# xarray-contrib/xeofs

Measured on AMD Instinct MI355X. Metric: EOF randomized-SVD GB/s (algorithmic: 16 passes x n x p x 4 B per fit / fit time), higher is better.
Workload: dtype f32 data, split-fp16 MFMA (f16x3+f16x3), f32 accumulate

## Files before the change

### xeofs_amd/csrc/eofx_abi.hip

```cpp
#include <chrono>
#include "eofx_hfft.hpp"
#include "eofx_kernels.hpp"
#include "eofx_fit.hpp"
#include "eofx_gram.hpp"
#include "eofx_axb_dma.hpp"
#include "eofx_hosteig.hpp"
#include "eofx_hostla.hpp"
#include "eofx_lag.hpp"
#include "eofx_gw.hpp"
#include "eofx_spca.hpp"
#include "eofx_lagcov.hpp"
#include "eofx_lowpass.hpp"
#include "eofx_orderpos.hpp"
#include "eofx_colquad.hpp"
#include "eofx_pairmin.hpp"
#include "eofx_spectral.hpp"
#include "eofx_pcmul.hpp"
#include "eofx_viewcov.hpp"
#include "eofx_lrfill.hpp"
#include "eofx_plans.hpp"
#include "eofx_sketch.hpp"
#include "eofx_hilbert_host.hpp"
#include "eofx_gwplan.hpp"
#ifndef EOFX_AXB_DMA_DEFAULT
#define EOFX_AXB_DMA_DEFAULT 1
#endif

#include <algorithm>
#include <array>
#include <atomic>
#include <cmath>
#include <complex>
#include <cstdarg>
#include <cstdio>
#include <cstring>
#include <functional>
#include <string>
#include <thread>
#include <mutex>
#include <shared_mutex>
#include <condition_variable>
#include <deque>
#include <memory>
#include <vector>

#include <dlfcn.h>
#include <pthread.h>
#include <sched.h>
#include <hipfft/hipfft.h>

#include "eofx.h"

using namespace eofx;

struct ncclUniqueIdCompat {
  char internal[128];
};

struct EofxComm {
  int world = 1, rank = 0;
  void* lib = nullptr;
  void* comm = nullptr;
  int (*p_allreduce)(const void*, void*, size_t, int, int, void*, hipStream_t) = nullptr;
  int (*p_destroy)(void*) = nullptr;
  const char* (*p_errstr)(int) = nullptr;
  eofx_allreduce_fn fn = nullptr;
  void* user = nullptr;
  int64_t calls = 0, bytes = 0;
  std::vector<std::pair<hipEvent_t, hipEvent_t>> events;
};

struct eofx_ctx {
  int device = 0;
  hipStream_t stream = nullptr;
  char* arena = nullptr;
  size_t arena_size = 0;
  size_t arena_off = 0;
  std::string err;
  int prec_power = EOFX_PREC_F16X3;
  int prec_final = EOFX_PREC_F16X3;
  std::vector<std::pair<void*, size_t>> pool;
  size_t pool_bytes = 0;
  size_t pool_cap = (size_t)160 << 30;
  struct HilbertSetup {
    int64_t n = 0, P = 0;
    int padding = 0;
    double decay = 0.0;
    void* chat = nullptr;
    float* hperm = nullptr;
    float* u = nullptr;
  };
  std::vector<HilbertSetup> hsetups;
  struct HilbertOp {
    int64_t n = 0;
    int padding = 0;
    double decay = 0.0;
    eofx_mat* m = nullptr;
  };
  std::vector<HilbertOp> hops;
  std::vector<std::pair<std::pair<int64_t, int64_t>, std::pair<void*, void*>>> fft_plans;
  int keep_raw = 0;
  bool allow_masked = false;
  bool want_rawT = false;
  float* pending_rawT = nullptr;
  size_t pending_rawT_bytes = 0;
  bool profile = false;
  struct ProfEvent {
    hipEvent_t first, second;
    int kind;
    ProfEvent(hipEvent_t a, hipEvent_t b, int k = 0) : first(a), second(b), kind(k) {}
  };
  std::vector<ProfEvent> prof_events;
  int64_t prof_kind_launches[3] = {0, 0, 0};
  double prof_kind_ms[3] = {0.0, 0.0, 0.0};
  double prof_flops = 0.0;
  double prof_bytes = 0.0;
  unsigned* amax_slots = nullptr;
  int amax_next = 0, amax_depth = 0;
  std::vector<std::pair<const float*, const unsigned*>> amax_known;
  double* pinned = nullptr;
  struct GramPlanDev {
    int nti = 0, ntj = 0, nst = 0;
    bool sym = false;
    GramPlan pl;
    GramItem* items = nullptr;
    int2* tiles = nullptr;
  };
  std::vector<GramPlanDev*> gram_plans;
  _Float16* axb_planes = nullptr;
  size_t axb_planes_bytes = 0;
  int axb_dma = -1;
  double fit_info[4] = {0.0, 0.0, 0.0, 0.0};
  int last_iters = 0;
  EofxComm* comm = nullptr;
};
constexpr int EOFX_AMAX_SLOTS = 1024;
constexpr int EOFX_HILBERT_OP_MAX_N = 16384;
constexpr size_t EOFX_PINNED_DOUBLES = 2 * 256 * 256 + 64;

struct eofx_mat {
  int64_t n = 0, p = 0, n_pad = 0, p_pad = 0;
  float* X = nullptr;
  float* Xt = nullptr;
  const float* raw = nullptr;
  float* raw_owned = nullptr;
  size_t raw_owned_bytes = 0;
  int64_t raw_ld = 0;
  float* aff = nullptr;
  unsigned* absmax_dev = nullptr;
  float absmax = 0.f;
  bool masked = false;
  int64_t p_valid = 0;
  int* act = nullptr;
  int64_t n_act = -1;
  float* rawT = nullptr;
};

static int set_err(eofx_ctx* ctx, int code, const char* fmt, ...) {
  char buf[512];
  va_list ap;
  va_start(ap, fmt);
  vsnprintf(buf, sizeof(buf), fmt, ap);
  va_end(ap);
  if (ctx) ctx->err = buf;
  return code;
}

#define HIPCHK(expr)                                                                          \
  do {                                                                                        \
    hipError_t _e = (expr);                                                                   \
    if (_e != hipSuccess)                                                                     \
      return set_err(ctx, _e == hipErrorOutOfMemory ? EOFX_ERR_NOMEM : EOFX_ERR_HIP,           \
                     "%s failed: %s (%s:%d)", #expr, hipGetErrorString(_e), __FILE__, __LINE__); \
// ... 92 lines not shown
    if (excl) {
      (void)hipStreamSynchronize(ctx->stream);
      g_fence[dev].mu.unlock();
    } else {
      g_fence[dev].mu.unlock_shared();
    }
  }
};
#define ENTER(c)          \
  FenceGuard _fence((c), false); \
  CHK(set_device(c))
#define ENTER_EXCLUSIVE(c)      \
  FenceGuard _fence((c), true); \
  CHK(set_device(c))

extern "C" int eofx_abi_version(void) { return EOFX_ABI_VERSION; }

extern "C" int eofx_ctx_create(int device, void* stream, eofx_ctx** out) {
  if (!out) return EOFX_ERR_ARG;
  eofx_ctx* ctx = new eofx_ctx();
  ctx->device = device;
  ctx->stream = (hipStream_t)stream;
  hipError_t e = hipSetDevice(device);
  if (e != hipSuccess) {
    delete ctx;
    *out = nullptr;
    return EOFX_ERR_HIP;
  }
  if (device >= 0 && device < EOFX_MAX_DEVICES) {
    std::lock_guard<std::mutex> g(g_fence[device].reg_mu);
    g_fence[device].ctxs.push_back(ctx);
  }
  *out = ctx;
  return EOFX_OK;
}
extern "C" int eofx_ctx_destroy(eofx_ctx* ctx) {
  if (!ctx) return EOFX_OK;
  {
    FenceGuard fence(ctx, false);
    if (ctx->device >= 0 && ctx->device < EOFX_MAX_DEVICES) {
      std::lock_guard<std::mutex> g(g_fence[ctx->device].reg_mu);
      auto& v = g_fence[ctx->device].ctxs;
      v.erase(std::remove(v.begin(), v.end(), ctx), v.end());
    }
  }
  (void)hipSetDevice(ctx->device);
  if (ctx->arena) {
    (void)hipStreamSynchronize(ctx->stream);
    (void)hipFree(ctx->arena);
  }
  pool_trim(ctx);
  if (ctx->amax_slots) (void)hipFree(ctx->amax_slots);
  if (ctx->pinned) (void)hipHostFree(ctx->pinned);
  for (auto& e : ctx->fft_plans) {
    hipfftDestroy((hipfftHandle)e.second.first);
    hipfftDestroy((hipfftHandle)e.second.second);
  }
  (void)eofx_ctx_comm_clear(ctx);
  if (ctx->axb_planes) (void)hipFree(ctx->axb_planes);
  for (auto* g : ctx->gram_plans) {
    if (g->items) (void)hipFree(g->items);
    if (g->tiles) (void)hipFree(g->tiles);
    delete g;
  }
  for (auto& h : ctx->hops) (void)eofx_mat_destroy(ctx, h.m);
  ctx->hops.clear();
  for (auto& h : ctx->hsetups) {
    if (h.chat) (void)hipFree(h.chat);
    if (h.hperm) (void)hipFree(h.hperm);
    if (h.u) (void)hipFree(h.u);
  }
  delete ctx;
  return EOFX_OK;
}
extern "C" int eofx_ctx_set_stream(eofx_ctx* ctx, void* stream) {
  if (!ctx) return EOFX_ERR_ARG;
  ENTER(ctx);
  if ((hipStream_t)stream == ctx->stream) return EOFX_OK;
  HIPCHK(hipStreamSynchronize(ctx->stream));
  ctx->stream = (hipStream_t)stream;
  for (auto& e : ctx->fft_plans) {
    if (hipfftSetStream((hipfftHandle)e.second.first, ctx->stream) != HIPFFT_SUCCESS ||
        hipfftSetStream((hipfftHandle)e.second.second, ctx->stream) != HIPFFT_SUCCESS)
      return set_err(ctx, EOFX_ERR_HIP, "hipfftSetStream failed while moving the context to another stream");
  }
  return EOFX_OK;
}
extern "C" int eofx_ctx_synchronize(eofx_ctx* ctx) {
  if (!ctx) return EOFX_ERR_ARG;
  ENTER(ctx);
  HIPCHK(hipStreamSynchronize(ctx->stream));
  return EOFX_OK;
}
extern "C" const char* eofx_last_error(const eofx_ctx* ctx) { return ctx ? ctx->err.c_str() : ""; }

extern "C" int eofx_ctx_profile(eofx_ctx* ctx, int enable) {
  if (!ctx) return EOFX_ERR_ARG;
  ctx->profile = enable != 0;
  return EOFX_OK;
}
extern "C" int eofx_ctx_profile_read(eofx_ctx* ctx, int64_t* launches, double* total_ms, double* flops,
                                     double* bytes) {
  if (!ctx) return EOFX_ERR_ARG;
  ENTER(ctx);
  HIPCHK(hipStreamSynchronize(ctx->stream));
  double ms = 0.0;
// ... 17 lines not shown
  ctx->prof_events.clear();
  ctx->prof_flops = 0.0;
  ctx->prof_bytes = 0.0;
  return EOFX_OK;
}

extern "C" int eofx_ctx_profile_by_kernel(const eofx_ctx* ctx, int64_t* launches3, double* ms3) {
  if (!ctx) return EOFX_ERR_ARG;
  for (int k = 0; k < 3; ++k) {
    if (launches3) launches3[k] = ctx->prof_kind_launches[k];
    if (ms3) ms3[k] = ctx->prof_kind_ms[k];
  }
  return EOFX_OK;
}

static int copy_out(eofx_ctx* ctx, void* dst, const void* src_dev, size_t bytes) {
  if (!dst || bytes == 0) return EOFX_OK;
  HIPCHK(hipMemcpyAsync(dst, src_dev, bytes, hipMemcpyDefault, ctx->stream));
  return EOFX_OK;
}
static int copy_in(eofx_ctx* ctx, void* dst_dev, const void* src, size_t bytes) {
  if (bytes == 0) return EOFX_OK;
  HIPCHK(hipMemcpyAsync(dst_dev, src, bytes, hipMemcpyDefault, ctx->stream));
  return EOFX_OK;
}

struct AmaxScope {
  eofx_ctx* ctx;
  explicit AmaxScope(eofx_ctx* c) : ctx(c) {
    if (ctx->amax_depth++ == 0) {
      ctx->amax_known.clear();
      ctx->amax_next = 0;
      if (!ctx->amax_slots && hipMalloc((void**)&ctx->amax_slots, sizeof(unsigned) * EOFX_AMAX_SLOTS) != hipSuccess) {
        (void)hipGetLastError();
        ctx->amax_slots = nullptr;
      }
      if (ctx->amax_slots &&
          hipMemsetAsync(ctx->amax_slots, 0, sizeof(unsigned) * EOFX_AMAX_SLOTS, ctx->stream) != hipSuccess) {
        (void)hipGetLastError();
        ctx->amax_next = EOFX_AMAX_SLOTS;
      }
    }
  }
  ~AmaxScope() {
    if (--ctx->amax_depth == 0) ctx->amax_known.clear();
  }
};
static void amax_forget(eofx_ctx* ctx, const float* panel) {
  for (size_t i = 0; i < ctx->amax_known.size(); ++i)
    if (ctx->amax_known[i].first == panel) {
      ctx->amax_known.erase(ctx->amax_known.begin() + i);
      return;
    }
}
static unsigned* amax_new(eofx_ctx* ctx, const float* panel) {
  if (ctx->amax_depth == 0) return nullptr;
  amax_forget(ctx, panel);
  if (!ctx->amax_slots || ctx->amax_next >= EOFX_AMAX_SLOTS) return nullptr;
  unsigned* slot = ctx->amax_slots + ctx->amax_next++;
  ctx->amax_known.emplace_back(panel, slot);
  return slot;
}
static const float* amax_get(const eofx_ctx* ctx, const float* panel) {
  if (ctx->amax_depth == 0) return nullptr;
  for (auto& e : ctx->amax_known)
    if (e.first == panel) return reinterpret_cast<const float*>(e.second);
  return nullptr;
}
static int pinned_scratch(eofx_ctx* ctx, double** out) {
  if (!ctx->pinned) HIPCHK(hipHostMalloc((void**)&ctx->pinned, sizeof(double) * EOFX_PINNED_DOUBLES, hipHostMallocDefault));
  *out = ctx->pinned;
  return EOFX_OK;
}

extern "C" int eofx_host_zheigh_top_f64(const double* Hr, const double* Hi, int m, int nev, double* w, double* Xr, double* Xi) {
  if (!Hr || !Hi || !w || !Xr || !Xi || m <= 0 || nev <= 0 || nev > m) return EOFX_ERR_ARG;
  return hosteig::zheigh_top(Hr, Hi, m, nev, w, Xr, Xi) == 0 ? EOFX_OK : EOFX_ERR_LINALG;
}
extern "C" int eofx_host_eigh_f64(const double* Ain, int n, double* w, double* Vec) {
  if (!Ain || !w || !Vec || n <= 0) return EOFX_ERR_ARG;
  return hosteig::eigh(Ain, n, w, Vec) == 0 ? EOFX_OK : EOFX_ERR_LINALG;
}


struct AffView {
  const float* aff = nullptr;
  int64_t ld = 0;
  int rows = 0;
  int64_t cols = 0;
  bool masked = false;
};
template <int NB>
static void launch_atb_variant(int prec, dim3 grid, hipStream_t st, const float* A, int64_t lda,
                               const float* B, int ldb, float* out, int L, int64_t M, int64_t K,
                               int64_t kps, int col_base, float a_scale, const float* b_absmax,
                               const AffView* aff = nullptr, const float* A2 = nullptr, const float* B2 = nullptr,
                               int s_half = 0, int sym = 0, unsigned* amax_out = nullptr, int l_valid = 128) {
  if (prec == EOFX_PREC_F16X3 && A2)
    hipLaunchKernelGGL(atb_f16_kernel<NB>, grid, dim3(256), 0, st, A, lda, B, ldb, out, L, M, K, kps, col_base,
                       a_scale, b_absmax, (const float*)nullptr, (int64_t)0, 0, (int64_t)0, A2, B2, s_half, 0, amax_out, l_valid);
  else if (prec == EOFX_PREC_F16X3 && aff && aff->masked)
    hipLaunchKernelGGL((atb_f16_kernel<NB, true, true>), grid, dim3(256), 0, st, A, lda, B, ldb, out, L, M, K, kps, col_base,
                       a_scale, b_absmax, aff->aff, aff->ld, aff->rows, aff->cols, (const float*)nullptr, (const float*)nullptr, 0, sym, amax_out,
                       l_valid);
  else if (prec == EOFX_PREC_F16X3 && aff)
    hipLaunchKernelGGL((atb_f16_kernel<NB, true>), grid, dim3(256), 0, st, A, lda, B, ldb, out, L, M, K, kps, col_base,
// ... 3283 lines not shown
};

static bool cplx_lean(const eofx_mat* A, const eofx_mat* B, int LP, int prec_power, int prec_final) {
  const bool all_written = A->X && A->Xt && B->X && B->Xt;
  return !all_written && !B->masked && LP == 64 && prec_power == EOFX_PREC_F16X3 && prec_final == EOFX_PREC_F16X3;
}
static int cplx_lean_setup(eofx_ctx* ctx, CplxOps& ops) {
  const int64_t n = ops.A->n, il = round_up(n, AXB_KG);
  float* ident = arena_alloc<float>(ctx, 3 * (size_t)il);
  if (!ident) return set_err(ctx, EOFX_ERR_NOMEM, "arena exhausted (identity map)");
  std::vector<float> h(3 * (size_t)il, 0.f);
  for (int64_t i = 0; i < n; ++i) h[2 * (size_t)il + i] = 1.f;
  CHK(copy_in(ctx, ident, h.data(), sizeof(float) * h.size()));
  HIPCHK(hipStreamSynchronize(ctx->stream));
  ops.lean = true;
  ops.ident = ident;
  ops.ident_ld = il;
  return EOFX_OK;
}

extern "C" int eofx_cmat_mul_f32(eofx_ctx* ctx, const eofx_mat* A, const eofx_mat* B, int conj_left, const float* Pin, int L,
                                 int final_pass, float* Pout) {
  if (!ctx || !A || !B || !Pin || !Pout) return set_err(ctx, EOFX_ERR_ARG, "bad argument");
  if (A->n != B->n || A->p != B->p) return set_err(ctx, EOFX_ERR_SHAPE, "real and imaginary parts must have the same shape");
  if (L != 64 && L != 128) return set_err(ctx, EOFX_ERR_ARG, "complex panels are 64 or 128 real columns wide");
  ENTER(ctx);
  const int prec = final_pass ? ctx->prec_final : ctx->prec_power;
  const bool lean = cplx_lean(A, B, L, prec, prec);
  if (!lean) {
    CHK(ensure_X(ctx, A));
    CHK(ensure_X(ctx, B));
  }
  const int64_t big = std::max(A->n_pad, A->p_pad);
  CHK(arena_reserve(ctx, c64_mul_scratch_bytes(A->n, A->p, A->n_pad, A->p_pad, L)));
  ArenaScope scope(ctx);
  ARENA(float, rot, (size_t)big * L);
  ARENA(float, tmp, (size_t)big * L);
  CplxOps ops{ctx, A, B, L, rot, tmp, std::max(A->absmax, B->absmax)};
  if (lean) CHK(cplx_lean_setup(ctx, ops));
  CHK(conj_left ? ops.zh_mul(Pin, Pout, prec) : ops.z_mul(Pin, Pout, prec));
  HIPCHK(hipStreamSynchronize(ctx->stream));
  return EOFX_OK;
}

struct C64Driver {
  eofx_ctx* const ctx;
  const eofx_mat* const A;
  const C64Plan pl;
  const int64_t p_total;
  const bool shd;
  const int l, LP;
  const int k, pp, pf;
  const bool trace;
  CplxOps ops{};
  float *Zs = nullptr, *Ws = nullptr, *Yt = nullptr, *Qt = nullptr, *Tv = nullptr, *Sv = nullptr;
  double *G = nullptr, *Ed = nullptr;
  float *Kw = nullptr, *Ww = nullptr, *Pt = nullptr, *Vs = nullptr;
  double *Cd = nullptr, *Ecd = nullptr, *Eall = nullptr, *Cf = nullptr;
  std::vector<double> hG, hE, hC, hCf, Hr, Hi, hEall, dref, ones;
  std::vector<zdouble> H, T, blk;
  std::vector<std::vector<zdouble>> ritz_raw;
  int nb = 0, nW = 0;
  bool exhausted = false, orth_always = false, orth_rest = false;
  std::vector<std::vector<zdouble>> Rf;
  std::vector<zdouble> Hqq;
  std::vector<double> Xr, Xi, wv;
  std::vector<float> hs;
  std::vector<double> sign;

  C64Driver(eofx_ctx* c, const eofx_mat* a, const C64Plan& plan, int64_t ptot, int k_)
      : ctx(c), A(a), pl(plan), p_total(ptot), shd(ptot > 0), l(plan.l), LP(plan.LP), k(k_), pp(c->prec_power), pf(c->prec_final),
        trace(std::getenv("EOFX_C64_TRACE") != nullptr), hG((size_t)LP * LP), dref(l), ones(l, 1.0), Rf(plan.nbmax), sign(k_, 1.0) {}

  template <typename T_>
  int take(T_*& ptr, size_t count, const char* name) {
    ptr = arena_alloc<T_>(ctx, count);
    return ptr ? EOFX_OK : set_err(ctx, EOFX_ERR_NOMEM, "internal: arena exhausted (%s)", name);
  }
  int allocate(const eofx_mat* B, const eofx_mat* Hop, bool lean) {
    float *rot = nullptr, *tmp = nullptr;
    CHK(take(Zs, (size_t)pl.small_pad * LP, "Zs"));
    CHK(take(Ws, (size_t)pl.small_pad * LP, "Ws"));
    CHK(take(Yt, (size_t)pl.tall_pad * LP, "Yt"));
    CHK(take(Qt, (size_t)pl.tall_pad * LP, "Qt"));
    CHK(take(rot, (size_t)pl.big * LP, "rot"));
    CHK(take(tmp, (size_t)pl.big * LP, "tmp"));
    CHK(take(Tv, (size_t)pl.tall_pad * pl.Lo, "Tv"));
    CHK(take(Sv, (size_t)pl.small_pad * pl.Lo, "Sv"));
    CHK(take(G, (size_t)LP * LP, "G"));
    CHK(take(Ed, (size_t)LP * LP, "Ed"));
    if (pl.krylov) {
      Kw = arena_alloc<float>(ctx, (size_t)pl.small_pad * pl.ldk);
      Ww = arena_alloc<float>(ctx, (size_t)pl.small_pad * pl.ldk);
      Pt = arena_alloc<float>(ctx, (size_t)pl.nbmax * pl.tall_pad * LP);
      Vs = arena_alloc<float>(ctx, (size_t)pl.small_pad * LP);
      Cd = arena_alloc<double>(ctx, (size_t)pl.nbmax * LP * LP);
      Ecd = arena_alloc<double>(ctx, (size_t)pl.nbmax * LP * LP);
      Eall = arena_alloc<double>(ctx, (size_t)pl.nbmax * LP * LP);
      Cf = arena_alloc<double>(ctx, (size_t)pl.nbmax * pl.nbmax * LP * LP);
      if (!Kw || !Ww || !Pt || !Vs || !Cd || !Ecd || !Eall || !Cf) return set_err(ctx, EOFX_ERR_NOMEM, "arena exhausted (block Krylov panels)");
    }
    ops = CplxOps{ctx, A, B, LP, rot, tmp, B ? std::max(A->absmax, B->absmax) : A->absmax};
    ops.Hop = B ? nullptr : Hop;
    if (lean) CHK(cplx_lean_setup(ctx, ops));
    return EOFX_OK;
  }
  int start(const float* omega, int omega_cols) {
    std::vector<float> host((size_t)pl.small * LP, 0.f);
    for (int64_t i = 0; i < pl.small; ++i)
      for (int j = 0; j < l; ++j) host[(size_t)i * LP + j] = omega[(size_t)i * omega_cols + j];
    CHK(import_panel(ctx, host.data(), pl.small, LP, Zs, pl.small_pad, LP));
    orth_always = (pl.adaptive && !pl.krylov) || orth_tall_rule(shd ? round_up(p_total, ATB_BM) : pl.tall_pad, LP, pp);
    orth_rest = orth_always;
    ctx->last_iters = 0;
    return EOFX_OK;
  }

  int fwd(const float* in, float* out, int prec) { return pl.transposed ? ops.zh_mul(in, out, prec) : ops.z_mul(in, out, prec); }
  int bwd(const float* in, float* out, int prec) {
    if (!pl.transposed) return ops.zh_mul(in, out, prec);
    CHK(ops.z_mul(in, out, prec));
    if (shd) {
      amax_forget(ctx, out);
      CHK(comm_allreduce(ctx, out, pl.small_pad * LP, 0, 0));
    }
    return EOFX_OK;
  }
  int gram_h(const float* P, int64_t rows_pad, bool tall_side = false) {
    CHK(launch_gram(ctx, P, rows_pad, LP, G));
    if (shd && tall_side) CHK(comm_allreduce(ctx, G, (int64_t)LP * LP, 1, 0));
    HIPCHK(hipMemcpyAsync(hG.data(), G, sizeof(double) * LP * LP, hipMemcpyDeviceToHost, ctx->stream));
    HIPCHK(hipStreamSynchronize(ctx->stream));
    if (!hostla::hermitian_from_real(hG.data(), LP, l, H))
      return set_err(ctx, EOFX_ERR_LINALG, "SVD failed. This may be due to isolated NaN values in the data.");
    return EOFX_OK;
  }
  int right_mul(const float* P, int64_t rows_pad, const std::vector<zdouble>& M, int mcols, int Lout, float* out, const double* colscale = nullptr) {
    hostla::embed_right(M.data(), l, l, mcols, LP, Lout, hE, colscale);
    HIPCHK(hipMemcpyAsync(Ed, hE.data(), sizeof(double) * LP * Lout, hipMemcpyHostToDevice, ctx->stream));
    CHK(launch_matmul(ctx, P, rows_pad, LP, Ed, Lout, out));
    HIPCHK(hipStreamSynchronize(ctx->stream));
    return EOFX_OK;
  }
  int orth(const float* P, int64_t rows_pad, float* out, bool tall_side = false) {
    CHK(gram_h(P, rows_pad, tall_side));
    hostla::chol_rinv(H.data(), l, l, T, 1e-13);
    return right_mul(P, rows_pad, T, l, LP, out);
  }
  int copy_block(float* wide, const float* src, int blk_) {
    HIPCHK(hipMemcpy2DAsync(wide + (size_t)blk_ * LP, sizeof(float) * pl.ldk, src, sizeof(float) * LP, sizeof(float) * LP, (size_t)pl.small_pad,
                            hipMemcpyDeviceToDevice, ctx->stream));
    return EOFX_OK;
  }
  int project(const float* Win, int nbk, float* out, bool to_host) {
    CHK(launch_xgram(ctx, Kw, pl.ldk, nbk * LP, Win, LP, LP, pl.small_pad, Cd));
    if (to_host) {
      hC.resize((size_t)nbk * LP * LP);
      HIPCHK(hipMemcpyAsync(hC.data(), Cd, sizeof(double) * hC.size(), hipMemcpyDeviceToHost, ctx->stream));
    }
    hipLaunchKernelGGL(cproj_embed_kernel, dim3((unsigned)std::min<int64_t>(((int64_t)nbk * pl.h * pl.h + 255) / 256, 1024)), dim3(256), 0, ctx->stream,
                       (const double*)Cd, nbk, LP, Ecd);
    KCHK();
    return launch_matmul_gen(ctx, Kw, pl.ldk, 64, 1 << 20, pl.small_pad, nbk * LP, Ecd, LP, Win, out);
  }
  int multiply_newest(std::vector<zdouble>* hqq) {
    float* slot = Pt + (size_t)nW * pl.tall_pad * LP;
    Rf[nW].clear();
    if (ctx->last_iters == 0 || orth_rest) {
      CHK(fwd(Zs, Yt, pp));
      CHK(gram_h(Yt, pl.tall_pad, true));
      if (hqq) *hqq = H;
      hostla::chol_rinv(H.data(), l, l, T, 1e-13, &Rf[nW]);
      return right_mul(Yt, pl.tall_pad, T, l, LP, slot);
    }
    CHK(fwd(Zs, slot, pp));
    if (hqq) {
      CHK(gram_h(slot, pl.tall_pad, true));
      *hqq = H;
    }
    return EOFX_OK;
  }
  int lanczos_step() {
    const int b = nW;
    CHK(multiply_newest(nullptr));
    CHK(bwd(Pt + (size_t)b * pl.tall_pad * LP, Ws, pp));
    const bool first = ctx->last_iters == 0;
    ++ctx->last_iters;
    CHK(copy_block(Ww, Ws, b));
    nW = b + 1;
    CHK(project(Ws, nb, Vs, true));
    CHK(gram_h(Vs, pl.small_pad));
    hostla::product_norms(H, hC.data(), nb, LP, l, dref);
    if (first && !orth_always && pl.n_iter > 1) {
      hostla::cplx_block(hC.data(), LP, pl.h, l, blk);
      std::vector<zdouble> H00 = Rf[0].empty() ? blk : hostla::zmatmul(blk, Rf[0], l), V0;
      hostla::hermitise(H00, l);
      std::vector<double> w0;
      orth_rest = hosteig::heigh(H00, l, w0, V0) != 0 || hostla::peaked_spectrum(w0.data(), l);
    }
    int live = 0;
    hostla::chol_rinv(H.data(), l, l, T, 1e-13, (std::vector<zdouble>*)nullptr, &live, dref.data(), 1e-10);
    CHK(right_mul(Vs, pl.small_pad, T, l, LP, Zs));
    if (live > 0) {
      CHK(project(Zs, nb, Vs, false));
      CHK(gram_h(Vs, pl.small_pad));
      hostla::chol_rinv(H.data(), l, l, T, 1e-13, (std::vector<zdouble>*)nullptr, &live, ones.data(), 0.25);
      CHK(right_mul(Vs, pl.small_pad, T, l, LP, Zs));
    }
    if (trace) fprintf(stderr, "[eofx_rsvd_c64] product %d: %d live columns in the next block (%d blocks)\n", ctx->last_iters, live, nb + (live > 0));
    if (live == 0) {
      exhausted = true;
      return EOFX_OK;
    }
    CHK(copy_block(Kw, Zs, nb));
    ++nb;
    return EOFX_OK;
  }
  int rayleigh_ritz(int nbr, bool with_last) {
    const int nWr = std::min(nW, nbr);
    CHK(launch_xgram(ctx, Kw, pl.ldk, nbr * LP, Ww, pl.ldk, nWr * LP, pl.small_pad, Cf));
    hCf.resize((size_t)nbr * LP * nWr * LP);
    HIPCHK(hipMemcpyAsync(hCf.data(), Cf, sizeof(double) * hCf.size(), hipMemcpyDeviceToHost, ctx->stream));
    HIPCHK(hipStreamSynchronize(ctx->stream));
    const int m = nbr * l;
    hostla::ritz_assemble(hCf.data(), nbr, nWr, nbr, LP, l, Rf, with_last ? &Hqq : nullptr, ritz_raw, Hr, Hi);
    if (!hostla::all_finite(Hr.data(), Hr.size())) return set_err(ctx, EOFX_ERR_LINALG, "SVD failed. This may be due to isolated NaN values in the data.");
    wv.assign(l, 0.0);
    Xr.assign((size_t)m * l, 0.0);
    Xi.assign((size_t)m * l, 0.0);
    const auto t_rr0 = std::chrono::steady_clock::now();
    const int rc_rr = hosteig::zheigh_top(Hr.data(), Hi.data(), m, l, wv.data(), Xr.data(), Xi.data());
    if (trace) fprintf(stderr, "[eofx_rsvd_c64] host Rayleigh-Ritz solve, order %d: %.2f ms\n", m,
                       1e3 * std::chrono::duration<double>(std::chrono::steady_clock::now() - t_rr0).count());
    if (rc_rr != 0 && hosteig::zheigh_top_embedded(Hr.data(), Hi.data(), m, l, wv.data(), Xr.data(), Xi.data()) != 0)
      return set_err(ctx, EOFX_ERR_LINALG, "complex SVD: Rayleigh-Ritz eigen-solver failed");
    return EOFX_OK;
  }
  int coeff_stack(int nbr, bool with_rf) {
    hEall.assign((size_t)nbr * LP * LP, 0.0);
    std::vector<double> eb;
    for (int b = 0; b < nbr; ++b) {
      const std::vector<zdouble> yb = hostla::ritz_block(Xr.data(), Xi.data(), b, l);
      const std::vector<zdouble> cb = (with_rf && !Rf[b].empty()) ? hostla::zmatmul(Rf[b], yb, l) : yb;
      hostla::embed_right(cb.data(), l, l, l, LP, LP, eb);
      std::copy(eb.begin(), eb.end(), hEall.begin() + (size_t)b * LP * LP);
    }
    HIPCHK(hipMemcpyAsync(Eall, hEall.data(), sizeof(double) * hEall.size(), hipMemcpyHostToDevice, ctx->stream));
    return EOFX_OK;
  }
  int compress() {
    const int nbr = nb - 1;
    CHK(rayleigh_ritz(nbr, false));
    if (trace) fprintf(stderr, "[eofx_rsvd_c64] thick restart after %d products: %d blocks -> Ritz block + newest block\n", ctx->last_iters, nb);
    CHK(coeff_stack(nbr, false));
    CHK(launch_matmul_gen(ctx, Kw, pl.ldk, 64, 1 << 20, pl.small_pad, nbr * LP, Eall, LP, nullptr, Vs));
    HIPCHK(hipStreamSynchronize(ctx->stream));
    CHK(coeff_stack(nbr, true));
    CHK(launch_matmul_gen(ctx, Ww, pl.ldk, 64, 1 << 20, pl.small_pad, nbr * LP, Eall, LP, nullptr, Ws));
    CHK(launch_matmul_gen(ctx, Pt, LP, pl.tall_pad * LP, LP / 64, pl.tall_pad, nbr * LP, Eall, LP, nullptr, Yt));
    HIPCHK(hipStreamSynchronize(ctx->stream));
    HIPCHK(hipMemcpyAsync(Pt, Yt, sizeof(float) * (size_t)pl.tall_pad * LP, hipMemcpyDeviceToDevice, ctx->stream));
    CHK(copy_block(Kw, Vs, 0));
    CHK(copy_block(Ww, Ws, 0));
    CHK(copy_block(Kw, Zs, 1));
    for (auto& rf : Rf) rf.clear();
    nb = 2;
    nW = 1;
    return EOFX_OK;
  }

  int range_krylov() {
    const int n_iter = pl.n_iter;
    CHK(orth(Zs, pl.small_pad, Vs));
    std::swap(Zs, Vs);
    CHK(copy_block(Kw, Zs, 0));
    nb = 1;
    hostla::RitzHistory history(pl.auto_count, C64_IT_MIN);
    while (ctx->last_iters < n_iter && !exhausted) {
      if (nb == pl.nbmax) CHK(compress());
      CHK(lanczos_step());
      if (pl.adaptive && !exhausted && ctx->last_iters >= history.next_check && ctx->last_iters < n_iter) {
        CHK(rayleigh_ritz(nb - 1, false));
        const bool stop = history.feed(wv.data(), k, l, ctx->last_iters, n_iter);
        if (trace) fprintf(stderr, "[eofx_rsvd_c64] after %d products: worst (error estimate / tolerance) over the leading %d Ritz values %.3e\n", ctx->last_iters, k, history.worst);
        if (stop) break;
        if (trace && history.factor > 0.0)
          fprintf(stderr, "[eofx_rsvd_c64] at this rate (x %.3g per %d products) the limit of %d products comes first: no further checks\n", history.factor, hostla::RitzHistory::check_every, n_iter);
      }
    }
    bool with_last = false;
    if (!exhausted) {
      CHK(multiply_newest(&Hqq));
      with_last = true;
    }
    CHK(rayleigh_ritz(nb, with_last));
    if (trace) fprintf(stderr, "[eofx_rsvd_c64] Rayleigh-Ritz over %d blocks (order %d) after %d products: leading Ritz values %.6e %.6e ... %.6e\n", nb, nb * l, ctx->last_iters, wv[0], l > 1 ? wv[1] : 0.0, wv[l - 1]);
    CHK(coeff_stack(nb, true));
    return launch_matmul_gen(ctx, Pt, LP, pl.tall_pad * LP, LP / 64, pl.tall_pad, nb * LP, Eall, LP, nullptr, Yt);
  }
  int range_subspace() {
    const int n_iter = pl.n_iter;
    std::vector<double> ritz_prev, w0;
    std::vector<zdouble> V0;
    int calm = 0;
    for (int it = 0; it < n_iter; ++it) {
      CHK(fwd(Zs, Yt, pp));
      if (it == 0 || orth_rest) {
        CHK(orth(Yt, pl.tall_pad, Qt, true));
        CHK(bwd(Qt, Ws, pp));
      } else {
        CHK(bwd(Yt, Ws, pp));
      }
      CHK(gram_h(Ws, pl.small_pad));
      ctx->last_iters = it + 1;
      if (it == 0 && !orth_always && n_iter > 1)
        orth_rest = hosteig::heigh(H, l, w0, V0) != 0 || hostla::peaked_spectrum(w0.data(), l);
      bool done = false;
      if (pl.adaptive && hosteig::heigh(H, l, w0, V0) == 0) {
        double worst = 0.0;
        if (ritz_prev.size() == (size_t)k)
          for (int j = 0; j < k; ++j) worst = std::max(worst, std::fabs(w0[j] - ritz_prev[j]) / std::max(w0[j], 1e-300));
        else
          worst = 1.0;
        ritz_prev.assign(w0.begin(), w0.begin() + k);
        calm = worst <= 1e-6 ? calm + 1 : 0;
        if (trace) fprintf(stderr, "[eofx_rsvd_c64] iteration %d: max relative change of the leading %d Ritz values %.3e\n", it + 1, k, worst);
        done = calm >= 2 && it + 1 >= C64_IT_MIN;
      }
      hostla::chol_rinv(H.data(), l, l, T, 1e-13);
      CHK(right_mul(Ws, pl.small_pad, T, l, LP, Zs));
      if (done) break;
    }
    return fwd(Zs, Yt, pp);
  }
  int final_stage() {
// ... 1356 lines not shown
```

### xeofs_amd/csrc/eofx_plans.hpp

```cpp
#pragma once
#include <algorithm>
#include <cmath>
#include <cstddef>
#include <cstdint>
#include <cstdlib>
#include <vector>

#include "eofx.h"

namespace eofx {

constexpr int ATB_KG = 32;
constexpr int ATB_BM = 512;
constexpr int AXB_KG = 64;
constexpr int AXB_BM = 256;
constexpr int GR_BM = 256;
constexpr int GR_BK = 32;
constexpr int64_t EOFX_GRAM_MAX_SIDE = 32768;
constexpr int SPCA_GMAX = 2048;
constexpr int VIEWCOV_T = 128;
constexpr int VIEWCOV_K = 16;
constexpr int VIEWCOV_WGS = 512;
constexpr int VIEWCOV_SPLIT_SLABS = 16;
constexpr int FIR_R = 64;
// ... 209 lines not shown
  bool adaptive;
  int n_iter, auto_count;
  int h, LP;
  int ko, Lo;
  bool transposed;
  int64_t small, small_pad, tall_pad, big;
  bool krylov;
  int nbmax;
  int64_t ldk;
  size_t arena_bytes;
};
inline C64Plan c64_plan(int64_t n, int64_t p, int64_t n_pad, int64_t p_pad, int64_t p_total, bool masked, int64_t p_valid, int k,
                        int n_oversamples, int n_iter, bool krylov_allowed) {
  C64Plan pl{};
  auto fail = [&](int status) { return pl.status = status, pl; };
  const bool shd = p_total > 0;
  if (shd && !(n < p_total)) return fail(C64_PLAN_SHARD_SIDE);
  pl.r = std::min(n, shd ? p_total : (masked ? p_valid : p));
  if (k > pl.r) return fail(C64_PLAN_RANK);
  pl.l = (int)std::min<int64_t>(k + n_oversamples, pl.r);
  if (pl.l > 64) return fail(C64_PLAN_WIDTH);
  if (!shd && masked && !(n < p_valid)) return fail(C64_PLAN_MASKED);
  pl.adaptive = n_iter == -2;
  pl.auto_count = k < 0.1 * (double)pl.r ? 7 : 4;
  if (n_iter == -1) n_iter = pl.auto_count;
  if (pl.adaptive) n_iter = C64_IT_CAP;
  if (n_iter < 0) return fail(C64_PLAN_N_ITER);
  pl.n_iter = n_iter;
  const int l = pl.l;
  pl.h = l <= 32 ? 32 : 64;
  pl.LP = 2 * pl.h;
  pl.ko = (int)round_up(k, 16);
  pl.Lo = 2 * pl.ko;
  pl.transposed = shd || n < p;
  pl.small = pl.transposed ? n : p;
  pl.small_pad = pl.transposed ? n_pad : p_pad;
  pl.tall_pad = pl.transposed ? p_pad : n_pad;
  pl.big = std::max(n_pad, p_pad);
  const int nb_fit = KRYLOV_MAX_ORDER / l;
  pl.krylov = n_iter >= 1 && nb_fit >= 3 && krylov_allowed;
  pl.nbmax = pl.krylov ? std::min(n_iter + 1, nb_fit) : 0;
  pl.ldk = (int64_t)pl.nbmax * pl.LP;
  const int LP = pl.LP, Lo = pl.Lo, nbmax = pl.nbmax;
  const int64_t small_pad = pl.small_pad, tall_pad = pl.tall_pad, big = pl.big;
  size_t need = (size_t)(2 * small_pad + 2 * tall_pad + 2 * big) * LP * 4 + (size_t)(small_pad + tall_pad) * Lo * 4;
  need += c64_pass_scratch_bytes(n, p, n_pad, p_pad, LP);
  need += (size_t)(4 * gram_parts(big, LP) + 8) * LP * LP * 8 + (size_t)big * (Lo + LP) * 4 + (8 << 20);
  if (pl.krylov)
    need += (size_t)nbmax * (2 * small_pad + tall_pad) * LP * 4 + (size_t)small_pad * LP * 4 + (size_t)(3 + nbmax) * nbmax * LP * LP * 8 +
            ((size_t)48 << 20);
  pl.arena_bytes = need;
  return pl;
}

inline int lag_groupsize(int E, int L) { return std::max(1, std::min(E, EOFX_LAG_GROUP_COLS / std::max(L, 1))); }
inline int lag_last_group(int E, int G) { return E - (E - 1) / G * G; }
inline int lag_blocks(int64_t total4) { return (int)std::max<int64_t>(1, std::min<int64_t>((total4 + 255) / 256, 8192)); }

inline int spca_grid(int64_t rows, int64_t entries) {
  const int64_t g = std::min<int64_t>(SPCA_GMAX, std::max<int64_t>(1, (rows + 127) / 128));
  const int64_t cap = std::max<int64_t>(1, ((int64_t)4 << 20) / std::max<int64_t>(1, entries));
  return (int)std::max<int64_t>(1, std::min(g, cap));
}

inline bool gram_fast_ok(int64_t n_pad, int64_t p, bool has_source) {
  return n_pad % GR_BM == 0 && n_pad <= EOFX_GRAM_MAX_SIDE && has_source && round_up(p, 2 * GR_BK) * 4 * GR_BM < ((int64_t)1 << 32) &&
         !std::getenv("EOFX_NO_FAST_GRAM");
}
inline bool tmul_nt_ok(int64_t n, int64_t p_pad, bool has_source, int L) {
  const int64_t kpad = round_up(n, 2 * GR_BK);
  return L >= 512 && p_pad % GR_BM == 0 && has_source && kpad * 4 * GR_BM < ((int64_t)1 << 32) && n >= 512 &&
         !std::getenv("EOFX_NO_TMUL_NT");
}
inline bool matmul_nt_ok(int64_t rows, int L, int Lo) {
  const int64_t kpad = round_up(L, 2 * GR_BK);
  return L >= 512 && Lo >= 256 && Lo % 4 == 0 && L % 4 == 0 && rows >= 1024 && rows % GR_BM == 0 &&
         kpad * 4 * GR_BM < ((int64_t)1 << 32) && !std::getenv("EOFX_NO_MATMUL_NT");
}
struct GramItem {
  int bi, bj, st0, nst, slot, pad0, pad1, pad2;
};
struct GramTile {
  int x, y;
};
struct GramPlan {
  int nti = 0, ntj = 0, T = 0, S = 1, st_per_split = 0, grid = 0;
  std::vector<GramItem> items;
  std::vector<GramTile> tiles;
};

inline unsigned gram_morton(unsigned i, unsigned j) {
  unsigned m = 0;
  for (int b = 0; b < 12; ++b) m |= ((i >> b) & 1u) << (2 * b + 1) | ((j >> b) & 1u) << (2 * b);
  return m;
}

inline void gram_plan_build(int nti, int ntj, bool sym, int nst_total, int S, GramPlan& pl) {
  pl.nti = nti;
  pl.ntj = ntj;
  pl.tiles.clear();
  for (int i = 0; i < nti; ++i)
    for (int j = sym ? i : 0; j < ntj; ++j) pl.tiles.push_back(GramTile{i, j});
  std::sort(pl.tiles.begin(), pl.tiles.end(), [](const GramTile& a, const GramTile& b) {
    return gram_morton((unsigned)a.x, (unsigned)a.y) < gram_morton((unsigned)b.x, (unsigned)b.y);
  });
  const int T = (int)pl.tiles.size();
// ... 148 lines not shown
```

Baseline: 5677.

## Overlap host Ritz solves with speculative forward pass and ring-buffered pinned uploads

Host-to-device coefficient uploads in the complex Lanczos driver now go through pinned ring buffers guarded by events, so the blocking stream synchronisations after right multiplies and compress steps can be dropped. During Rayleigh-Ritz at thick restarts and convergence checks, the next block's forward pass is queued on the GPU before the host eigen-solve runs, so device work overlaps host linear algebra. After a restart the speculated product is copied into its new slot. This adds pinned memory and event bookkeeping, plus correctness risk if a speculated product or slot is misused. The old behaviour is reachable by setting an environment variable.

```diff
diff --git a/xeofs_amd/csrc/eofx_abi.hip b/xeofs_amd/csrc/eofx_abi.hip
--- a/xeofs_amd/csrc/eofx_abi.hip
+++ b/xeofs_amd/csrc/eofx_abi.hip
@@ -69,6 +69,10 @@
   int64_t calls = 0, bytes = 0;
   std::vector<std::pair<hipEvent_t, hipEvent_t>> events;
 };
+
+constexpr int C64_RMUL_RING = 4;
+constexpr int C64_COEFF_RING = 2;
+constexpr int C64_STAGE_EVENTS = C64_RMUL_RING + C64_COEFF_RING;
 
 struct eofx_ctx {
   int device = 0;
@@ -119,6 +123,9 @@
   int amax_next = 0, amax_depth = 0;
   std::vector<std::pair<const float*, const unsigned*>> amax_known;
   double* pinned = nullptr;
+  double* c64_pin = nullptr;
+  size_t c64_pin_doubles = 0;
+  hipEvent_t c64_ev[C64_STAGE_EVENTS] = {};
   struct GramPlanDev {
     int nti = 0, ntj = 0, nst = 0;
     bool sym = false;
@@ -317,6 +324,9 @@
   pool_trim(ctx);
   if (ctx->amax_slots) (void)hipFree(ctx->amax_slots);
   if (ctx->pinned) (void)hipHostFree(ctx->pinned);
+  if (ctx->c64_pin) (void)hipHostFree(ctx->c64_pin);
+  for (hipEvent_t ev : ctx->c64_ev)
+    if (ev) (void)hipEventDestroy(ev);
   for (auto& e : ctx->fft_plans) {
     hipfftDestroy((hipfftHandle)e.second.first);
     hipfftDestroy((hipfftHandle)e.second.second);
@@ -440,6 +450,11 @@
       ctx->amax_known.erase(ctx->amax_known.begin() + i);
       return;
     }
+}
+static void amax_move(eofx_ctx* ctx, const float* from, const float* to) {
+  amax_forget(ctx, to);
+  for (auto& e : ctx->amax_known)
+    if (e.first == from) e.first = to;
 }
 static unsigned* amax_new(eofx_ctx* ctx, const float* panel) {
   if (ctx->amax_depth == 0) return nullptr;
@@ -3829,13 +3844,19 @@
   const int l, LP;
   const int k, pp, pf;
   const bool trace;
+  const bool speculate;
   CplxOps ops{};
   float *Zs = nullptr, *Ws = nullptr, *Yt = nullptr, *Qt = nullptr, *Tv = nullptr, *Sv = nullptr;
   double *G = nullptr, *Ed = nullptr;
   float *Kw = nullptr, *Ww = nullptr, *Pt = nullptr, *Vs = nullptr;
   double *Cd = nullptr, *Ecd = nullptr, *Eall = nullptr, *Cf = nullptr;
-  std::vector<double> hG, hE, hC, hCf, Hr, Hi, hEall, dref, ones;
+  std::vector<double> hE, Hr, Hi, hEall, dref, ones;
   std::vector<zdouble> H, T, blk;
+  double *hG = nullptr, *hC = nullptr, *hCf = nullptr;
+  double* hEs[C64_RMUL_RING] = {};
+  double* hEalls[C64_COEFF_RING] = {};
+  bool ev_live[C64_STAGE_EVENTS] = {};
+  int e_next = 0, c_next = 0;
   std::vector<std::vector<zdouble>> ritz_raw;
   int nb = 0, nW = 0;
   bool exhausted = false, orth_always = false, orth_rest = false;
@@ -3844,10 +3865,17 @@
   std::vector<double> Xr, Xi, wv;
   std::vector<float> hs;
   std::vector<double> sign;
-
+  bool spec = false;
+  float* spec_slot = nullptr;
+  const char* spec_under = "";
+
+  static bool speculate_env() {
+    const char* e = std::getenv("EOFX_C64_SPECULATE");
+    return !(e && atoi(e) == 0);
+  }
   C64Driver(eofx_ctx* c, const eofx_mat* a, const C64Plan& plan, int64_t ptot, int k_)
       : ctx(c), A(a), pl(plan), p_total(ptot), shd(ptot > 0), l(plan.l), LP(plan.LP), k(k_), pp(c->prec_power), pf(c->prec_final),
-        trace(std::getenv("EOFX_C64_TRACE") != nullptr), hG((size_t)LP * LP), dref(l), ones(l, 1.0), Rf(plan.nbmax), sign(k_, 1.0) {}
+        trace(std::getenv("EOFX_C64_TRACE") != nullptr), speculate(speculate_env()), dref(l), ones(l, 1.0), Rf(plan.nbmax), sign(k_, 1.0) {}
 
   template <typename T_>
   int take(T_*& ptr, size_t count, const char* name) {
@@ -3880,6 +3908,35 @@
     ops = CplxOps{ctx, A, B, LP, rot, tmp, B ? std::max(A->absmax, B->absmax) : A->absmax};
     ops.Hop = B ? nullptr : Hop;
     if (lean) CHK(cplx_lean_setup(ctx, ops));
+    return stage();
+  }
+  int stage() {
+    const size_t q = (size_t)LP * LP, nbm = (size_t)pl.nbmax;
+    const size_t need = q * (1 + C64_RMUL_RING + nbm + nbm * nbm + C64_COEFF_RING * nbm);
+    if (ctx->c64_pin_doubles < need) {
+      HIPCHK(hipStreamSynchronize(ctx->stream));
+      if (ctx->c64_pin) HIPCHK(hipHostFree(ctx->c64_pin));
+      ctx->c64_pin = nullptr;
+      ctx->c64_pin_doubles = 0;
+      HIPCHK(hipHostMalloc((void**)&ctx->c64_pin, sizeof(double) * need, hipHostMallocDefault));
+      ctx->c64_pin_doubles = need;
+    }
+    for (hipEvent_t& ev : ctx->c64_ev)
+      if (!ev) HIPCHK(hipEventCreateWithFlags(&ev, hipEventDisableTiming));
+    double* at = ctx->c64_pin;
+    hG = at, at += q;
+    for (double*& s : hEs) s = at, at += q;
+    hC = at, at += nbm * q;
+    hCf = at, at += nbm * nbm * q;
+    for (double*& s : hEalls) s = at, at += nbm * q;
+    return EOFX_OK;
+  }
+  int upload(double* host_slot, int ev_i, const std::vector<double>& src, size_t count, double* dev) {
+    if (ev_live[ev_i]) HIPCHK(hipEventSynchronize(ctx->c64_ev[ev_i]));
+    std::memcpy(host_slot, src.data(), sizeof(double) * count);
+    HIPCHK(hipMemcpyAsync(dev, host_slot, sizeof(double) * count, hipMemcpyHostToDevice, ctx->stream));
+    HIPCHK(hipEventRecord(ctx->c64_ev[ev_i], ctx->stream));
+    ev_live[ev_i] = true;
     return EOFX_OK;
   }
   int start(const float* omega, int omega_cols) {
@@ -3906,18 +3963,17 @@
   int gram_h(const float* P, int64_t rows_pad, bool tall_side = false) {
     CHK(launch_gram(ctx, P, rows_pad, LP, G));
     if (shd && tall_side) CHK(comm_allreduce(ctx, G, (int64_t)LP * LP, 1, 0));
-    HIPCHK(hipMemcpyAsync(hG.data(), G, sizeof(double) * LP * LP, hipMemcpyDeviceToHost, ctx->stream));
+    HIPCHK(hipMemcpyAsync(hG, G, sizeof(double) * LP * LP, hipMemcpyDeviceToHost, ctx->stream));
     HIPCHK(hipStreamSynchronize(ctx->stream));
-    if (!hostla::hermitian_from_real(hG.data(), LP, l, H))
+    if (!hostla::hermitian_from_real(hG, LP, l, H))
       return set_err(ctx, EOFX_ERR_LINALG, "SVD failed. This may be due to isolated NaN values in the data.");
     return EOFX_OK;
   }
   int right_mul(const float* P, int64_t rows_pad, const std::vector<zdouble>& M, int mcols, int Lout, float* out, const double* colscale = nullptr) {
     hostla::embed_right(M.data(), l, l, mcols, LP, Lout, hE, colscale);
-    HIPCHK(hipMemcpyAsync(Ed, hE.data(), sizeof(double) * LP * Lout, hipMemcpyHostToDevice, ctx->stream));
-    CHK(launch_matmul(ctx, P, rows_pad, LP, Ed, Lout, out));
-    HIPCHK(hipStreamSynchronize(ctx->stream));
-    return EOFX_OK;
+    const int slot = e_next++ % C64_RMUL_RING;
+    CHK(upload(hEs[slot], slot, hE, (size_t)LP * Lout, Ed));
+    return launch_matmul(ctx, P, rows_pad, LP, Ed, Lout, out);
   }
   int orth(const float* P, int64_t rows_pad, float* out, bool tall_side = false) {
     CHK(gram_h(P, rows_pad, tall_side));
@@ -3931,26 +3987,35 @@
   }
   int project(const float* Win, int nbk, float* out, bool to_host) {
     CHK(launch_xgram(ctx, Kw, pl.ldk, nbk * LP, Win, LP, LP, pl.small_pad, Cd));
-    if (to_host) {
-      hC.resize((size_t)nbk * LP * LP);
-      HIPCHK(hipMemcpyAsync(hC.data(), Cd, sizeof(double) * hC.size(), hipMemcpyDeviceToHost, ctx->stream));
-    }
+    if (to_host) HIPCHK(hipMemcpyAsync(hC, Cd, sizeof(double) * (size_t)nbk * LP * LP, hipMemcpyDeviceToHost, ctx->stream));
     hipLaunchKernelGGL(cproj_embed_kernel, dim3((unsigned)std::min<int64_t>(((int64_t)nbk * pl.h * pl.h + 255) / 256, 1024)), dim3(256), 0, ctx->stream,
                        (const double*)Cd, nbk, LP, Ecd);
     KCHK();
     return launch_matmul_gen(ctx, Kw, pl.ldk, 64, 1 << 20, pl.small_pad, nbk * LP, Ecd, LP, Win, out);
   }
+  int speculate_newest(const char* under) {
+    if (spec || !c64_speculation_ok(speculate, orth_rest, ctx->last_iters, pl.n_iter, exhausted)) return EOFX_OK;
+    spec_slot = Pt + (size_t)nW * pl.tall_pad * LP;
+    spec_under = under;
+    CHK(fwd(Zs, spec_slot, pp));
+    spec = true;
+    return EOFX_OK;
+  }
   int multiply_newest(std::vector<zdouble>* hqq) {
     float* slot = Pt + (size_t)nW * pl.tall_pad * LP;
     Rf[nW].clear();
     if (ctx->last_iters == 0 || orth_rest) {
+      if (spec) return set_err(ctx, EOFX_ERR_ARG, "internal: a product was queued ahead on the orthonormalising route");
       CHK(fwd(Zs, Yt, pp));
       CHK(gram_h(Yt, pl.tall_pad, true));
       if (hqq) *hqq = H;
       hostla::chol_rinv(H.data(), l, l, T, 1e-13, &Rf[nW]);
       return right_mul(Yt, pl.tall_pad, T, l, LP, slot);
     }
-    CHK(fwd(Zs, slot, pp));
+    if (spec && spec_slot != slot) return set_err(ctx, EOFX_ERR_ARG, "internal: the product queued ahead is not in the block's slot");
+    if (!spec) CHK(fwd(Zs, slot, pp));
+    else if (trace) fprintf(stderr, "[eofx_rsvd_c64] speculated forward pass of block %d under %s: consumed by %s\n", nb - 1, spec_under, hqq ? "the stop branch" : "the next step");
+    spec = false;
     if (hqq) {
       CHK(gram_h(slot, pl.tall_pad, true));
       *hqq = H;
@@ -3967,13 +4032,14 @@
     nW = b + 1;
     CHK(project(Ws, nb, Vs, true));
     CHK(gram_h(Vs, pl.small_pad));
-    hostla::product_norms(H, hC.data(), nb, LP, l, dref);
+    hostla::product_norms(H, hC, nb, LP, l, dref);
     if (first && !orth_always && pl.n_iter > 1) {
-      hostla::cplx_block(hC.data(), LP, pl.h, l, blk);
+      hostla::cplx_block(hC, LP, pl.h, l, blk);
       std::vector<zdouble> H00 = Rf[0].empty() ? blk : hostla::zmatmul(blk, Rf[0], l), V0;
       hostla::hermitise(H00, l);
       std::vector<double> w0;
       orth_rest = hosteig::heigh(H00, l, w0, V0) != 0 || hostla::peaked_spectrum(w0.data(), l);
+      if (trace && orth_rest) fprintf(stderr, "[eofx_rsvd_c64] peaked spectrum: the tall panel is orthonormalised in the remaining products\n");
     }
     int live = 0;
     hostla::chol_rinv(H.data(), l, l, T, 1e-13, (std::vector<zdouble>*)nullptr, &live, dref.data(), 1e-10);
@@ -3993,14 +4059,14 @@
     ++nb;
     return EOFX_OK;
   }
-  int rayleigh_ritz(int nbr, bool with_last) {
+  int rayleigh_ritz(int nbr, bool with_last, const char* ahead = nullptr) {
     const int nWr = std::min(nW, nbr);
     CHK(launch_xgram(ctx, Kw, pl.ldk, nbr * LP, Ww, pl.ldk, nWr * LP, pl.small_pad, Cf));
-    hCf.resize((size_t)nbr * LP * nWr * LP);
-    HIPCHK(hipMemcpyAsync(hCf.data(), Cf, sizeof(double) * hCf.size(), hipMemcpyDeviceToHost, ctx->stream));
+    HIPCHK(hipMemcpyAsync(hCf, Cf, sizeof(double) * (size_t)nbr * LP * nWr * LP, hipMemcpyDeviceToHost, ctx->stream));
     HIPCHK(hipStreamSynchronize(ctx->stream));
+    if (ahead) CHK(speculate_newest(ahead));
     const int m = nbr * l;
-    hostla::ritz_assemble(hCf.data(), nbr, nWr, nbr, LP, l, Rf, with_last ? &Hqq : nullptr, ritz_raw, Hr, Hi);
+    hostla::ritz_assemble(hCf, nbr, nWr, nbr, LP, l, Rf, with_last ? &Hqq : nullptr, ritz_raw, Hr, Hi);
     if (!hostla::all_finite(Hr.data(), Hr.size())) return set_err(ctx, EOFX_ERR_LINALG, "SVD failed. This may be due to isolated NaN values in the data.");
     wv.assign(l, 0.0);
     Xr.assign((size_t)m * l, 0.0);
@@ -4022,20 +4088,18 @@
       hostla::embed_right(cb.data(), l, l, l, LP, LP, eb);
       std::copy(eb.begin(), eb.end(), hEall.begin() + (size_t)b * LP * LP);
     }
-    HIPCHK(hipMemcpyAsync(Eall, hEall.data(), sizeof(double) * hEall.size(), hipMemcpyHostToDevice, ctx->stream));
-    return EOFX_OK;
+    const int slot = c_next++ % C64_COEFF_RING;
+    return upload(hEalls[slot], C64_RMUL_RING + slot, hEall, hEall.size(), Eall);
   }
   int compress() {
     const int nbr = nb - 1;
-    CHK(rayleigh_ritz(nbr, false));
+    CHK(rayleigh_ritz(nbr, false, "the solve of a thick restart"));
     if (trace) fprintf(stderr, "[eofx_rsvd_c64] thick restart after %d products: %d blocks -> Ritz block + newest block\n", ctx->last_iters, nb);
     CHK(coeff_stack(nbr, false));
     CHK(launch_matmul_gen(ctx, Kw, pl.ldk, 64, 1 << 20, pl.small_pad, nbr * LP, Eall, LP, nullptr, Vs));
-    HIPCHK(hipStreamSynchronize(ctx->stream));
     CHK(coeff_stack(nbr, true));
     CHK(launch_matmul_gen(ctx, Ww, pl.ldk, 64, 1 << 20, pl.small_pad, nbr * LP, Eall, LP, nullptr, Ws));
     CHK(launch_matmul_gen(ctx, Pt, LP, pl.tall_pad * LP, LP / 64, pl.tall_pad, nbr * LP, Eall, LP, nullptr, Yt));
-    HIPCHK(hipStreamSynchronize(ctx->stream));
     HIPCHK(hipMemcpyAsync(Pt, Yt, sizeof(float) * (size_t)pl.tall_pad * LP, hipMemcpyDeviceToDevice, ctx->stream));
     CHK(copy_block(Kw, Vs, 0));
     CHK(copy_block(Ww, Ws, 0));
@@ -4043,6 +4107,13 @@
     for (auto& rf : Rf) rf.clear();
     nb = 2;
     nW = 1;
+    if (spec) {
+      float* slot = Pt + (size_t)nW * pl.tall_pad * LP;
+      HIPCHK(hipMemcpyAsync(slot, spec_slot, sizeof(float) * (size_t)pl.tall_pad * LP, hipMemcpyDeviceToDevice, ctx->stream));
+      amax_move(ctx, spec_slot, slot);
+      spec_slot = slot;
+      if (trace) fprintf(stderr, "[eofx_rsvd_c64] thick restart: the forward pass queued under %s moves to slot 1\n", spec_under);
+    }
     return EOFX_OK;
   }
 
@@ -4057,7 +4128,7 @@
       if (nb == pl.nbmax) CHK(compress());
       CHK(lanczos_step());
       if (pl.adaptive && !exhausted && ctx->last_iters >= history.next_check && ctx->last_iters < n_iter) {
-        CHK(rayleigh_ritz(nb - 1, false));
+        CHK(rayleigh_ritz(nb - 1, false, "a convergence check"));
         const bool stop = history.feed(wv.data(), k, l, ctx->last_iters, n_iter);
         if (trace) fprintf(stderr, "[eofx_rsvd_c64] after %d products: worst (error estimate / tolerance) over the leading %d Ritz values %.3e\n", ctx->last_iters, k, history.worst);
         if (stop) break;
diff --git a/xeofs_amd/csrc/eofx_plans.hpp b/xeofs_amd/csrc/eofx_plans.hpp
--- a/xeofs_amd/csrc/eofx_plans.hpp
+++ b/xeofs_amd/csrc/eofx_plans.hpp
@@ -285,6 +285,9 @@
   pl.arena_bytes = need;
   return pl;
 }
+inline bool c64_speculation_ok(bool enabled, bool orth_rest, int products, int limit, bool exhausted) {
+  return enabled && !orth_rest && products > 0 && products < limit && !exhausted;
+}
 
 inline int lag_groupsize(int E, int L) { return std::max(1, std::min(E, EOFX_LAG_GROUP_COLS / std::max(L, 1))); }
 inline int lag_last_group(int E, int G) { return E - (E - 1) / G * G; }
```

Result: no change. 5632 (-0.8%).
